# Z1HaoC/YOLO-Dual

Measured on AMD Instinct MI355X. Metric: images/sec at 640x640 bs=16/GPU, higher is better.
Workload: dtype bf16; 1 GPU; YOLOv5-backbone (C3+SPPF) + UNet-lite SegmentHead, fwd+bwd+SGD/EMA step, 640x640, bs=16/GPU, CE+0.5*Dice, 12 classes (BASELINE configs[1]); global_batch=16, parallelism=dp1

## Files before the change

yolo_dual_amd/csrc/igemm.hip:

```cpp
#include "conv_common.h"

#define GROWB 128


struct IgemmArgs {
    const void* A;
    const void* B;
    void* C;
    float* stats;
    int N, Hi, Wi, lda;
    int Kc;
    int Ho, Wo, ldc;
    int Cout;
    int Cst;
    int Hg, Wg;
    int in_mul, out_mul, out_h0, out_w0;
    int ntaps, Ttot;
    int accumulate;
    int M;
    int stats_ld;
    int stats_atomic;
    unsigned bytesA, bytesB;
    unsigned bytesC;
    unsigned ldb_bytes;
// ... 1167 lines not shown
#pragma unroll
            for (int j = 0; j < PT; ++j) bfr[j] = *(const uint4*)(pst + prow[j] * GROWB + ((kq ^ ((prow[j] >> 1) & 7)) << 4));
#pragma unroll
            for (int c = 0; c < CT; ++c)
#pragma unroll
                for (int j = 0; j < PT; ++j) Mma<T>::run(af[c], bfr[j], acc[c][j]);
        }
        stg = stg + 1 == S ? 0 : stg + 1;
    };
#define H_STEPS(F, CB)                                                                                                          \
    step(std::integral_constant<int, 0>{}, F, CB); step(std::integral_constant<int, 1>{}, F, CB);                              \
    step(std::integral_constant<int, 2>{}, F, CB); step(std::integral_constant<int, 3>{}, F, CB);                              \
    step(std::integral_constant<int, 4>{}, F, CB); step(std::integral_constant<int, 5>{}, F, CB);                              \
    step(std::integral_constant<int, 6>{}, F, CB); step(std::integral_constant<int, 7>{}, F, CB);                              \
    step(std::integral_constant<int, 8>{}, F, CB)
    H_STEPS(std::true_type{}, 0);
    for (int cb = 1; cb < spt; ++cb) { H_STEPS(std::false_type{}, cb); }
#undef H_STEPS
    asm volatile("s_waitcnt lgkmcnt(0)" ::: "memory");
    wait_vm_barrier<0>();
    igemm2_epilogue<BM, BN, NW, WP>(p, acc, smem, 0, n0, mtile, BM, 16, 8, n * p.Ho + h0, w0);
}

#define HS_PROWS 184
template <int BN, int NW, int WP, bool ONEP = false>
__global__ __launch_bounds__(NW * 64) void igemm2hs_kernel(const IgemmArgs p) {
    using T = bf16_t;
    constexpr int ES = 2;
    constexpr int BM = 128;
    constexpr int RPP = NW * 8;
    constexpr int BR = BN / RPP;
    constexpr int PP = (HS_PROWS + RPP - 1) / RPP;
    constexpr int WN = NW / WP;
    constexpr int BNW = BN / WN;
    constexpr int CT = BNW / 16;
    constexpr int PT = BM / (16 * WP);
    constexpr int PBYTES = HS_PROWS * GROWB;
    constexpr int RBYTES = BN * GROWB;
    static_assert(BN % RPP == 0 && (ONEP ? 1 : 2) * PBYTES + 2 * RBYTES >= BM * BN * 2 + 8192, "stage geometry");
    extern __shared__ __attribute__((aligned(16))) unsigned char smem[];
    constexpr int NPB = ONEP ? 1 : 2;
    unsigned char* const ring = smem + NPB * PBYTES;
    int* const sTd = (int*)(ring + 2 * RBYTES);
    int* const sTw = sTd + 16;
    const int t = threadIdx.x;
    if (t < 9) {
        sTd[t] = (int)p.dh[t] * H_PW + (int)p.dw[t];
        sTw[t] = (int)p.wt[t] * p.Kc * ES;
    }
    __syncthreads();
    const int lane = t & 63;
    const int wave = __builtin_amdgcn_readfirstlane(t >> 6);
    const int wc = wave % WN, wp = wave / WN;
    const int tile = xcd_remap(blockIdx.x, gridDim.x);
    int mtile, ntile;
    if (p.m_fastest) { ntile = tile / p.grid_m; mtile = tile - ntile * p.grid_m; }
    else { mtile = tile / p.grid_n; ntile = tile - mtile * p.grid_n; }
    const int tiles_w = p.Wo >> 4, tiles_hw = (p.Ho >> 3) * tiles_w;
    const int n = mtile / tiles_hw;
    const int rem = mtile - n * tiles_hw;
    const int h0 = (rem / tiles_w) << 3, w0 = (rem % tiles_w) << 4;
    const int n0 = ntile * BN;
    const int r = t >> 3, qs = t & 7;
    unsigned poff[PP];
#pragma unroll
    for (int i = 0; i < PP; ++i) {
        const int rho = r + RPP * i;
        const int pr = rho / H_PW, pc = rho - pr * H_PW;
        const int h = h0 - 1 + pr, w = w0 - 1 + pc;
        const bool ok = rho < 10 * H_PW && (unsigned)h < (unsigned)p.Hi && (unsigned)w < (unsigned)p.Wi;
        poff[i] = ok ? (unsigned)(((n * p.Hi + h) * p.Wi + w) * p.lda) * (unsigned)ES + (unsigned)((qs ^ ((rho >> 1) & 7)) << 4) : 0xFFFFFFFFu;
    }
    unsigned browoff[BR];
#pragma unroll
    for (int i = 0; i < BR; ++i) {
        const int row = r + RPP * i;
        const int co = n0 + row;
        browoff[i] = co < p.Cout ? (unsigned)co * p.ldb_bytes + (unsigned)((qs ^ ((row >> 1) & 7)) << 4) : 0xF0000000u;
    }
    const int spt = p.Kc >> 6;
    const int nsteps = 9 * spt;
    u32x4 rsA, rsB;
    ring_rsrc(p, rsA, rsB);
    const unsigned lds0 = (unsigned)(size_t)(__attribute__((address_space(3))) unsigned char*)smem;
    const unsigned wave_lds = lds0 + (unsigned)wave * (8 * GROWB);
    auto issue_patch = [&](int cb) {
        const unsigned base = wave_lds + (unsigned)(ONEP ? 0 : (cb & 1)) * PBYTES;
        const unsigned kb = (unsigned)cb << 7;
#pragma unroll
        for (int i = 0; i < PP; ++i) {
            if (RPP * i + wave * 8 < HS_PROWS)
                lds_dma16(rsA, base + i * RPP * GROWB, poff[i] == 0xFFFFFFFFu ? 0xFFFFFFFFu : poff[i] + kb);
        }
    };
    auto issue_w = [&](int stg, int cbw, int woff) {
        const unsigned add = cbw < spt ? (unsigned)woff + ((unsigned)cbw << 7) : 0xF0000000u;
        const unsigned base = wave_lds + (unsigned)NPB * PBYTES + (unsigned)stg * RBYTES;
#pragma unroll
        for (int i = 0; i < BR; ++i) lds_dma16(rsB, base + i * RPP * GROWB, browoff[i] + add);
    };
    f32x4 acc[CT][PT];
#pragma unroll
    for (int c = 0; c < CT; ++c)
#pragma unroll
        for (int j = 0; j < PT; ++j) acc[c][j] = f32x4{0.f, 0.f, 0.f, 0.f};
    const int lrow = lane & 15, lgrp = lane >> 4;
    const int sw_w = (lrow >> 1) & 7;
    const unsigned char* const fa = ring + (wc * BNW + lrow) * GROWB;
    issue_patch(0);
    issue_w(0, 0, sTw[0]);
    int cb = 0, tap = 0;
    int dcur = sTd[0], wnx = sTw[1];
    for (int g = 0; g < nsteps; ++g) {
        asm volatile("s_waitcnt lgkmcnt(0)" ::: "memory");
        wait_vm_barrier<0>();
        const int t1 = tap == 8 ? 0 : tap + 1, c1 = tap == 8 ? cb + 1 : cb;
        const int t2 = t1 == 8 ? 0 : t1 + 1;
        const int dnx = sTd[t1], wnn = sTw[t2];
        issue_w((g + 1) & 1, c1, wnx);
        if constexpr (ONEP) {
            if (tap == 0 && cb > 0) {
                issue_patch(cb);
                wait_vm_barrier<0>();
            }
        } else {
            if (tap == 0 && cb + 1 < spt) issue_patch(cb + 1);
        }
        const unsigned char* const wst = fa + (g & 1) * RBYTES;
        const unsigned char* const pst = smem + (ONEP ? 0 : (cb & 1)) * PBYTES;
        int prow[PT];
#pragma unroll
        for (int j = 0; j < PT; ++j) prow[j] = (wp * PT + j + 1) * H_PW + (lrow + 1) + dcur;
#pragma unroll
        for (int half = 0; half < 2; ++half) {
            uint4 af[CT], bfr[PT];
            const int kq = lgrp + 4 * half;
#pragma unroll
            for (int c = 0; c < CT; ++c) af[c] = *(const uint4*)(wst + c * 16 * GROWB + ((kq ^ sw_w) << 4));
#pragma unroll
            for (int j = 0; j < PT; ++j) bfr[j] = *(const uint4*)(pst + prow[j] * GROWB + ((kq ^ ((prow[j] >> 1) & 7)) << 4));
#pragma unroll
            for (int c = 0; c < CT; ++c)
#pragma unroll
                for (int j = 0; j < PT; ++j) Mma<T>::run(af[c], bfr[j], acc[c][j]);
        }
        dcur = dnx; wnx = wnn; tap = t1; cb = c1;
    }
    asm volatile("s_waitcnt lgkmcnt(0)" ::: "memory");
    wait_vm_barrier<0>();
    igemm2_epilogue<BM, BN, NW, WP>(p, acc, smem, 0, n0, mtile, BM, 16, 8, n * p.Ho + h0, w0);
}

#define WR_PW 34
typedef __attribute__((ext_vector_type(16))) float f32x16_t;
template <int CO, bool STATS, int NW>
__global__ __launch_bounds__(NW * 64, 2) void igemm2w_kernel(const IgemmArgs p, int nblocks) {
    using T = bf16_t;
    constexpr int CG = CO / 32, PG = NW / CG, RW = 2, R = PG * RW;
    constexpr int NT = NW * 64, PR = NW * 8;
    constexpr int PROWS = (R + 2) * WR_PW;
    constexpr int PASSES = (PROWS + PR - 1) / PR;
    constexpr int PBYTES = PASSES * PR * GROWB;
    constexpr int BPX = R * 32;
    constexpr int NCH = CO / 8;
    constexpr int ORB = CO * 2;
    static_assert(BPX * NCH == 4 * NT && NT % NCH == 0, "four 16-byte store slots per thread, a fixed channel chunk per thread");
    extern __shared__ __attribute__((aligned(16))) unsigned char smem[];
    unsigned char* const stage = smem + 2 * PBYTES;
    float* const sred = (float*)smem;
    const int t = threadIdx.x, lane = t & 63;
    const int wave = __builtin_amdgcn_readfirstlane(t >> 6);
    const int cg = wave % CG, pg = wave / CG;
    const int ln = lane & 31, lh = lane >> 5;
    const int blocks_w = p.Wo >> 5, blocks_img = (p.Ho / R) * blocks_w;
    const u32x4 rsA = buf_rsrc(p.A, p.bytesA), rsC = buf_rsrc(p.C, p.bytesC);
    const unsigned lds0 = (unsigned)(size_t)(__attribute__((address_space(3))) unsigned char*)smem;
    const unsigned wave_lds = lds0 + (unsigned)wave * 1024u;
    const int rq = t >> 3, qs = t & 7;
    int pprc[PASSES];
#pragma unroll
    for (int i = 0; i < PASSES; ++i) {
        const int rho = i * PR + rq;
        pprc[i] = rho < PROWS ? ((rho / WR_PW) << 8) | (rho - (rho / WR_PW) * WR_PW) : (4000000 << 8);
    }
    auto block_origin = [&](int b, int& n, int& h0, int& w0) {
        n = b / blocks_img;
        const int rem = b - n * blocks_img;
        h0 = (rem / blocks_w) * R;
        w0 = (rem % blocks_w) << 5;
    };
    auto issue_patch = [&](int b, int buf) {
        int n, h0, w0;
        block_origin(b, n, h0, w0);
        const bool live = b < nblocks;
#pragma unroll
        for (int i = 0; i < PASSES; ++i) {
            const int rho = i * PR + rq;
            const int h = h0 - 1 + (pprc[i] >> 8), w = w0 - 1 + (pprc[i] & 255);
            const bool ok = live && (unsigned)h < (unsigned)p.Hi && (unsigned)w < (unsigned)p.Wi;
            const unsigned off = (unsigned)(((n * p.Hi + h) * p.Wi + w) * p.lda) * 2u + (unsigned)((qs ^ ((rho >> 1) & 7)) << 4);
            lds_dma16(rsA, wave_lds + (unsigned)buf * PBYTES + (unsigned)(i * PR * GROWB), ok ? off : 0xFFFFFFFFu);
        }
    };
    const int per = (nblocks + (int)gridDim.x - 1) / (int)gridDim.x;
    const int b0 = blockIdx.x * per, b1 = min(nblocks, b0 + per);
    issue_patch(b0, 0);
    uint4 wreg[9][4];
    {
        const __amdgpu_buffer_rsrc_t rsB = __builtin_amdgcn_make_buffer_rsrc((void*)p.B, 0, p.bytesB, 0x00020000);
        const int co = cg * 32 + ln;
#pragma unroll
        for (int tp = 0; tp < 9; ++tp)
#pragma unroll
            for (int ks = 0; ks < 4; ++ks) {
                const unsigned off = co < p.Cout ? (unsigned)co * p.ldb_bytes + (unsigned)(((int)p.wt[tp] * p.Kc + ks * 16 + lh * 8) * 2) : 0xFFFFFFFFu;
                const u32x4 v = __builtin_amdgcn_raw_buffer_load_b128(rsB, off, 0, 0);
                wreg[tp][ks] = make_uint4(v.x, v.y, v.z, v.w);
            }
    }
    int tapd[9];
#pragma unroll
    for (int tp = 0; tp < 9; ++tp) tapd[tp] = (int)p.dh[tp] * WR_PW + (int)p.dw[tp];
    float s1[STATS ? 16 : 1], s2[STATS ? 16 : 1];
#pragma unroll
    for (int e = 0; e < (STATS ? 16 : 1); ++e) { s1[e] = 0.f; s2[e] = 0.f; }
    const bool want_stats = STATS && p.stats != nullptr;
    int ridx_base = (pg * RW + 1) * WR_PW + ln + 1;
    asm volatile("s_waitcnt vmcnt(0)\n\ts_barrier" ::: "memory");
    int buf = 0;
    for (int b = b0; b < b1; ++b, buf ^= 1) {
        issue_patch(b + 1 < b1 ? b + 1 : nblocks, buf ^ 1);
        const unsigned char* const pst = smem + buf * PBYTES;
        f32x16_t acc[RW];
#pragma unroll
        for (int rb = 0; rb < RW; ++rb)
#pragma unroll
            for (int e = 0; e < 16; ++e) acc[rb][e] = 0.f;
        asm volatile("" : "+v"(ridx_base));
        uint4 fq[2][4];
        auto rd = [&](int tp, int rb, uint4 (&f)[4]) {
            const int ridx = ridx_base + rb * WR_PW + tapd[tp];
            const unsigned char* const rowp = pst + ridx * GROWB;
            const int sw = (ridx >> 1) & 7;
#pragma unroll
            for (int ks = 0; ks < 4; ++ks) f[ks] = *(const uint4*)(rowp + (((2 * ks + lh) ^ sw) << 4));
        };
        rd(0, 0, fq[0]);
#pragma unroll
        for (int step = 0; step < 9 * RW; ++step) {
            const int tp = step / RW, rb = step % RW;
            if (step + 1 < 9 * RW) rd((step + 1) / RW, (step + 1) % RW, fq[(step + 1) & 1]);
#pragma unroll
            for (int ks = 0; ks < 4; ++ks)
                acc[rb] = __builtin_amdgcn_mfma_f32_32x32x16_bf16(__builtin_bit_cast(bf16x8, wreg[tp][ks]),
                                                                  __builtin_bit_cast(bf16x8, fq[step & 1][ks]), acc[rb], 0, 0, 0);
            __builtin_amdgcn_sched_barrier(0);
        }
        if constexpr (STATS) {
            if (want_stats) {
#pragma unroll
                for (int rb = 0; rb < RW; ++rb)
#pragma unroll
                    for (int e = 0; e < 16; ++e) { s1[e] += acc[rb][e]; s2[e] = fmaf(acc[rb][e], acc[rb][e], s2[e]); }
            }
        }
#pragma unroll
        for (int rb = 0; rb < RW; ++rb) {
            const int px = (pg * RW + rb) * 32 + ln;
#pragma unroll
            for (int g = 0; g < 4; ++g) {
                uint2 u;
                u.x = (uint32_t)f2bf(acc[rb][4 * g + 0]) | ((uint32_t)f2bf(acc[rb][4 * g + 1]) << 16);
                u.y = (uint32_t)f2bf(acc[rb][4 * g + 2]) | ((uint32_t)f2bf(acc[rb][4 * g + 3]) << 16);
                const int chq = cg * 4 + g;
                *(uint2*)(stage + px * ORB + ((chq ^ (px & (NCH - 1))) << 4) + (lh << 3)) = u;
            }
        }
        asm volatile("s_waitcnt lgkmcnt(0)\n\ts_barrier" ::: "memory");
        {
            int n, h0, w0;
            block_origin(b, n, h0, w0);
#pragma unroll
            for (int j = 0; j < 4; ++j) {
                const int idx = t + NT * j;
                const int px = idx / NCH, ch = idx % NCH;
                const uint4 v = *(const uint4*)(stage + px * ORB + ((ch ^ (px & (NCH - 1))) << 4));
                const unsigned m = (unsigned)((n * p.Ho + h0 + (px >> 5)) * p.Wo + w0 + (px & 31));
                const unsigned off = ch * 8 < p.Cst ? (m * (unsigned)p.ldc + (unsigned)(ch * 8)) * 2u : 0xFFFFFFFFu;
                asm volatile("s_waitcnt lgkmcnt(0)" ::: "memory");
                buf_store16_asm(u32x4{v.x, v.y, v.z, v.w}, off, rsC);
            }
        }
        asm volatile("s_waitcnt vmcnt(4)\n\ts_barrier" ::: "memory");
    }
    if constexpr (!STATS) {
        asm volatile("s_waitcnt vmcnt(0)" ::: "memory");
        return;
    }
    if (want_stats) {
#pragma unroll
        for (int e = 0; e < (STATS ? 16 : 1); ++e)
#pragma unroll
            for (int o = 1; o < 32; o <<= 1) { s1[e] += __shfl_xor(s1[e], o, 64); s2[e] += __shfl_xor(s2[e], o, 64); }
        asm volatile("s_waitcnt vmcnt(0) lgkmcnt(0)\n\ts_barrier" ::: "memory");
        if (ln == 0) {
#pragma unroll
            for (int e = 0; e < (STATS ? 16 : 1); ++e) {
                const int c = cg * 32 + (e >> 2) * 8 + lh * 4 + (e & 3);
                sred[(pg * CO + c) * 2] = s1[e];
                sred[(pg * CO + c) * 2 + 1] = s2[e];
            }
        }
        __syncthreads();
        if (t < CO && t < p.Cout) {
            float a = 0.f, b2 = 0.f;
#pragma unroll
            for (int w = 0; w < PG; ++w) { a += sred[(w * CO + t) * 2]; b2 += sred[(w * CO + t) * 2 + 1]; }
            float* dst = p.stats + (size_t)(blockIdx.x & (YDL_BN_REPLICAS - 1)) * 2 * p.stats_ld;
            atomicAdd(dst + t, a);
            atomicAdd(dst + p.stats_ld + t, b2);
        }
    } else {
        asm volatile("s_waitcnt vmcnt(0)" ::: "memory");
    }
}

static int g_wreg = 1;
static bool wreg_ok(const IgemmArgs& a) {
    if (!g_wreg || a.accumulate) return false;
    if (a.ncls > 1 || a.ntaps != 9 || a.Ttot != 9 || a.in_mul != 1 || a.out_mul != 1 || a.out_h0 != 0 || a.out_w0 != 0) return false;
    if (a.Hi != a.Ho || a.Wi != a.Wo || a.Hg != a.Ho || a.Wg != a.Wo || a.Kc != 64) return false;
    if (a.Cst != 64 && a.Cst != 128) return false;
    if ((a.Wo & 31) || a.Ho % (a.Cst == 128 ? 4 : 8)) return false;
    if (a.stats != nullptr && !a.stats_atomic) return false;
    if ((long long)a.M < 4ll * 128 * ydl_device_cus()) return false;
    bool seen[9] = {false, false, false, false, false, false, false, false, false};
    for (int t = 0; t < 9; ++t) {
        const int dh = a.dh[t], dw = a.dw[t];
        if (dh < -1 || dh > 1 || dw < -1 || dw > 1 || seen[(dh + 1) * 3 + dw + 1]) return false;
        seen[(dh + 1) * 3 + dw + 1] = true;
    }
    return true;
}
template <int CO>
static int launch_igemm2w_cfg(IgemmArgs a, hipStream_t st, int fam) {
    constexpr int NW = 4, R = (NW / (CO / 32)) * 2, PR = NW * 8;
    const int nblocks = a.N * (a.Ho / R) * (a.Wo >> 5);
    constexpr int PASSES = ((R + 2) * WR_PW + PR - 1) / PR;
    const size_t smem = 2 * (size_t)PASSES * PR * GROWB + (size_t)R * 32 * CO * 2;
    YDL_SET_MAX_LDS((igemm2w_kernel<CO, true, NW>), smem);
    YDL_SET_MAX_LDS((igemm2w_kernel<CO, false, NW>), smem);
    const unsigned long long bc = ((unsigned long long)(a.N * a.Ho * a.Wo - 1) * a.ldc + a.Cst) * 2ull;
    YDL_CHECK(bc < 0xFFFFFFF0ull, "output larger than 4 GiB");
    a.bytesC = (unsigned)bc;
    ydl_note_kernel(fam, CO == 128 ? "igemm2w_kernel<128,nw4>" : "igemm2w_kernel<64,nw4>");
    const int ctas = std::min(ydl_device_cus() * 2, nblocks);
    if (a.stats != nullptr) igemm2w_kernel<CO, true, NW><<<ctas, NW * 64, smem, st>>>(a, nblocks);
    else igemm2w_kernel<CO, false, NW><<<ctas, NW * 64, smem, st>>>(a, nblocks);
    YDL_LAUNCH_CHECK();
    return 0;
}
static int launch_igemm2w(const IgemmArgs& a, hipStream_t st, int fam) {
    return a.Cst == 128 ? launch_igemm2w_cfg<128>(a, st, fam) : launch_igemm2w_cfg<64>(a, st, fam);
}

#define S2_PW 17
#define S2_PROWS 192
__device__ constexpr int kS2Kh[9] = {1, 1, 2, 2, 1, 2, 0, 0, 0};
__device__ constexpr int kS2Kw[9] = {1, 2, 1, 2, 0, 0, 1, 2, 0};
template <int NW, int WP, int S, bool ACC>
__global__ __launch_bounds__(NW * 64, NW / 2) void igemm2s_kernel(const IgemmArgs p) {
    using T = bf16_t;
    constexpr int ES = 2;
    constexpr int BM = 128, BN = 64;
    constexpr int RPP = NW * 8;
    constexpr int BR = BN / RPP;
    constexpr int PP = (S2_PROWS + RPP - 1) / RPP;
    constexpr int WN = NW / WP;
    constexpr int BNW = BN / WN;
    constexpr int CT = BNW / 16;
    constexpr int PT = BM / (16 * WP);
    constexpr int PBYTES = S2_PROWS * GROWB;
    constexpr int RBYTES = BN * GROWB;
    static_assert(BN % RPP == 0 && BR == 1 && S2_PROWS % RPP == 0 && (S == 2 || S == 3), "one weight DMA per thread and step, whole patch passes");
    static_assert(2 * PBYTES + S * RBYTES >= BM * BN * 2, "epilogue scratch");
    extern __shared__ __attribute__((aligned(16))) unsigned char smem[];
    unsigned char* const ring = smem + 2 * PBYTES;
    const int t = threadIdx.x;
    const int lane = t & 63;
    const int wave = __builtin_amdgcn_readfirstlane(t >> 6);
    const int wc = wave % WN, wp = wave / WN;
    const int tile = xcd_remap(blockIdx.x, gridDim.x);
    const int mtile = tile / p.grid_n, ntile = tile - mtile * p.grid_n;
    const int tiles_w = p.Wi >> 4, tiles_hw = (p.Hi >> 3) * tiles_w;
    const int n = mtile / tiles_hw;
    const int rem = mtile - n * tiles_hw;
    const int i0 = (rem / tiles_w) << 3, j0 = (rem % tiles_w) << 4;
    const int n0 = ntile * BN;
    const int r = t >> 3, qs = t & 7;
    const unsigned browoff = (n0 + r) < p.Cout ? (unsigned)(n0 + r) * p.ldb_bytes + (unsigned)((qs ^ ((r >> 1) & 7)) << 4) : 0xF0000000u;
    const int spt = p.Kc >> 6;
    u32x4 rsA, rsB;
    ring_rsrc(p, rsA, rsB);
    const unsigned lds0 = (unsigned)(size_t)(__attribute__((address_space(3))) unsigned char*)smem;
    const unsigned wave_lds = lds0 + (unsigned)wave * (8 * GROWB);
    auto issue_patch = [&](int cb) {
        const unsigned base = wave_lds + (unsigned)(cb & 1) * PBYTES;
        const unsigned kb = (unsigned)cb << 7;
        const bool live = cb < spt;
#pragma unroll
        for (int i = 0; i < PP; ++i) {
            const int rho = r + RPP * i;
            const int pr = rho / S2_PW, pc = rho - pr * S2_PW;
            const int h = i0 + pr, w = j0 + pc;
            const bool ok = live && rho < 9 * S2_PW && h < p.Hi && w < p.Wi;
            const unsigned off = (unsigned)(((n * p.Hi + h) * p.Wi + w) * p.lda) * (unsigned)ES + (unsigned)((qs ^ ((rho >> 1) & 7)) << 4) + kb;
            lds_dma16(rsA, base + i * RPP * GROWB, ok ? off : 0xFFFFFFFFu);
        }
    };
    auto issue_w = [&](int stg, int cb, int slice) {
        const unsigned add = cb < spt ? (unsigned)slice * (unsigned)p.Kc * ES + ((unsigned)cb << 7) : 0xF0000000u;
        lds_dma16(rsB, wave_lds + 2u * PBYTES + (unsigned)stg * RBYTES, browoff + add);
    };
    f32x4 acc[4][CT][PT];
#pragma unroll
    for (int q = 0; q < 4; ++q)
#pragma unroll
        for (int c = 0; c < CT; ++c)
#pragma unroll
            for (int j = 0; j < PT; ++j) acc[q][c][j] = f32x4{0.f, 0.f, 0.f, 0.f};
    const int lrow = lane & 15, lgrp = lane >> 4;
    const int sw_w = (lrow >> 1) & 7;
    const unsigned char* const fa = ring + (wc * BNW + lrow) * GROWB;
    uint4 bq[2][PT];
    auto step = [&](auto ic, int cb) {
        constexpr int I = decltype(ic)::value;
        constexpr int kh = kS2Kh[I], kw = kS2Kw[I];
        constexpr int dh = kh == 0 ? 1 : 0, dw = kw == 0 ? 1 : 0;
        constexpr int cls = (kh != 1 ? 2 : 0) + (kw != 1 ? 1 : 0);
        constexpr bool group_start = I == 0 || I == 4 || I == 6 || I == 8;
        constexpr int I1 = (I + 8) % 9, I2 = (I + 7) % 9;
        constexpr int NY = S == 2 ? 0 : 1 + (I1 == 0 ? PP : 0) + (I2 == 0 ? PP : 0);
        asm volatile("s_waitcnt lgkmcnt(0)" ::: "memory");
        wait_vm_barrier<NY>();
        {
            constexpr int J = (I + S - 1) % 9;
            const int cbj = cb + (I + S - 1) / 9;
            issue_w(S == 3 ? J % 3 : (cbj + J) & 1, cbj, kS2Kh[J] * 3 + kS2Kw[J]);
        }
        if constexpr (I == 0) issue_patch(cb + 1);
        const unsigned char* const wst = fa + (S == 3 ? I % 3 : (cb + I) & 1) * RBYTES;
        const unsigned char* const pst = smem + (cb & 1) * PBYTES;
        if constexpr (group_start) {
#pragma unroll
            for (int j = 0; j < PT; ++j) {
                const int prow = (wp * PT + j + dh) * S2_PW + (lrow + dw);
                const unsigned char* const rowp = pst + prow * GROWB;
                const int sw = (prow >> 1) & 7;
                bq[0][j] = *(const uint4*)(rowp + ((lgrp ^ sw) << 4));
                bq[1][j] = *(const uint4*)(rowp + (((lgrp + 4) ^ sw) << 4));
            }
        }
#pragma unroll
        for (int half = 0; half < 2; ++half) {
            uint4 aq[CT];
#pragma unroll
            for (int c = 0; c < CT; ++c) aq[c] = *(const uint4*)(wst + c * 16 * GROWB + (((lgrp + 4 * half) ^ sw_w) << 4));
#pragma unroll
            for (int c = 0; c < CT; ++c)
#pragma unroll
                for (int j = 0; j < PT; ++j) Mma<T>::run(aq[c], bq[half][j], acc[cls][c][j]);
        }
    };
    issue_patch(0);
    issue_w(0, 0, kS2Kh[0] * 3 + kS2Kw[0]);
    if constexpr (S == 3) issue_w(1, 0, kS2Kh[1] * 3 + kS2Kw[1]);
    for (int cb = 0; cb < spt; ++cb) {
        step(std::integral_constant<int, 0>{}, cb); step(std::integral_constant<int, 1>{}, cb); step(std::integral_constant<int, 2>{}, cb);
        step(std::integral_constant<int, 3>{}, cb); step(std::integral_constant<int, 4>{}, cb); step(std::integral_constant<int, 5>{}, cb);
        step(std::integral_constant<int, 6>{}, cb); step(std::integral_constant<int, 7>{}, cb); step(std::integral_constant<int, 8>{}, cb);
    }
    asm volatile("s_waitcnt lgkmcnt(0)" ::: "memory");
    wait_vm_barrier<0>();
    if constexpr (ACC) {
        constexpr int CPR = BN / 8, RPS = NW * 64 / CPR, ORB = BN * 2;
        static_assert(4 * BM * ORB <= 2 * PBYTES + S * RBYTES && CPR == 8, "the four previous tiles must fit the LDS");
        const u32x4 rsC = buf_rsrc(p.C, p.bytesC);
#pragma unroll
        for (int q = 0; q < 4; ++q)
#pragma unroll
            for (int i = 0; i < BM / RPS; ++i) {
                const int row = r + i * RPS;
                const int gh = row >> 4, gw = row & 15;
                const unsigned pix = (unsigned)((n * p.Ho + 2 * (i0 + gh) + (q >> 1)) * p.Wo + 2 * (j0 + gw) + (q & 1));
                const int co = n0 + ((qs ^ (row & 7)) << 3);
                lds_dma16(rsC, wave_lds + (unsigned)(q * BM * ORB + i * RPS * ORB), co < p.Cst ? (pix * (unsigned)p.ldc + (unsigned)co) * ES : 0xFFFFFFFFu);
                __builtin_amdgcn_sched_barrier(0);
            }
        wait_vm_barrier<0>();
#pragma unroll
        for (int q = 0; q < 4; ++q)
#pragma unroll
            for (int j = 0; j < PT; ++j) {
                const int row = wp * (BM / WP) + j * 16 + lrow;
#pragma unroll
                for (int c = 0; c < CT; ++c) {
                    const int ch = wc * BNW + c * 16 + lgrp * 4;
                    const uint2 q2 = *(const uint2*)(smem + q * BM * ORB + row * ORB + ((((ch >> 3) ^ (row & 7))) << 4) + ((ch & 4) << 1));
                    acc[q][c][j] += f32x4{__uint_as_float(q2.x << 16), __uint_as_float(q2.x & 0xffff0000u),
                                          __uint_as_float(q2.y << 16), __uint_as_float(q2.y & 0xffff0000u)};
                }
                __builtin_amdgcn_sched_barrier(0);
            }
        __syncthreads();
    }
// ... 630 lines not shown
}

template <int BM, int BN, int NW, int WP, int S, int NL>
static int launch_igemm2l(IgemmArgs a, hipStream_t st, int fam) {
    if (int e = ring_grid(a, BM, BN)) return e;
    const size_t smem = (size_t)S * (BM + BN) * GROWB + 3 * MAXTAPS * sizeof(int);
    static const std::string nm = std::string("igemm2l_kernel<") + std::to_string(BM) + "," + std::to_string(BN) + "," + std::to_string(NW) + "+" +
                                  std::to_string(NL) + "," + std::to_string(S) + ">";
    YDL_SET_MAX_LDS((igemm2l_kernel<BM, BN, NW, WP, S, NL>), smem);
    ydl_note_kernel(fam, nm.c_str());
    igemm2l_kernel<BM, BN, NW, WP, S, NL><<<dim3(a.grid_m * a.grid_n), (NW + NL) * 64, smem, st>>>(a);
    YDL_LAUNCH_CHECK();
    return 0;
}

static int g_halo = 1;
static bool halo_ok(const IgemmArgs& a, int id) {
    if (!g_halo || !kRing[id].patch) return false;
    if (a.ncls > 1 || a.ntaps != 9 || a.Ttot != 9 || a.in_mul != 1 || a.out_mul != 1 || a.out_h0 != 0 || a.out_w0 != 0) return false;
    if (a.Hi != a.Ho || a.Wi != a.Wo || a.Hg != a.Ho || a.Wg != a.Wo || (a.Ho & 7) || (a.Wo & 15) || (a.Kc & 63)) return false;
    bool seen[9] = {false, false, false, false, false, false, false, false, false};
    for (int t = 0; t < 9; ++t) {
        const int dh = a.dh[t], dw = a.dw[t];
        if (dh < -1 || dh > 1 || dw < -1 || dw > 1 || seen[(dh + 1) * 3 + dw + 1]) return false;
        seen[(dh + 1) * 3 + dw + 1] = true;
    }
    return true;
}
template <int BN, int S>
static int launch_igemm2h(IgemmArgs a, hipStream_t st, int fam) {
    constexpr int NW = 8, WP = 4;
    if (int e = ring_grid(a, 128, BN)) return e;
    static const std::string nm = std::string("igemm2h_kernel<128,") + std::to_string(BN) + "," + std::to_string(S) + ">";
    ydl_note_kernel(fam, nm.c_str());
    if constexpr (S == 2) {
        if (a.Kc == 64) {
            const size_t smem = (size_t)HS_PROWS * GROWB + 2 * (size_t)BN * GROWB + 128;
            YDL_SET_MAX_LDS((igemm2hs_kernel<BN, NW, WP, true>), smem);
            igemm2hs_kernel<BN, NW, WP, true><<<dim3(a.grid_m * a.grid_n), NW * 64, smem, st>>>(a);
        } else {
            const size_t smem = 2 * (size_t)HS_PROWS * GROWB + 2 * (size_t)BN * GROWB + 128;
            YDL_SET_MAX_LDS((igemm2hs_kernel<BN, NW, WP>), smem);
            igemm2hs_kernel<BN, NW, WP><<<dim3(a.grid_m * a.grid_n), NW * 64, smem, st>>>(a);
        }
    } else {
        const size_t smem = 2 * (size_t)H_PROWS * GROWB + (size_t)S * BN * GROWB;
        YDL_SET_MAX_LDS((igemm2h_kernel<BN, NW, WP, S>), smem);
        igemm2h_kernel<BN, NW, WP, S><<<dim3(a.grid_m * a.grid_n), NW * 64, smem, st>>>(a);
    }
    YDL_LAUNCH_CHECK();
    return 0;
}
static int launch_patch(int id, const IgemmArgs& a, hipStream_t st, int fam) {
    if (kRing[id].BN == 128) return launch_igemm2h<128, 2>(a, st, fam);
    if (a.Kc == 64) return launch_igemm2h<64, 2>(a, st, fam);
    return launch_igemm2h<64, 3>(a, st, fam);
}

static int g_s2fused = 1;
static bool s2fused_ok(const ydl_conv_geom* g, int dtype) {
    if (!g_s2fused || !g_ring_enabled || dtype != YDL_BF16) return false;
    if (g->k != 3 || g->s != 2 || g->p != 1 || g->Hi != 2 * g->Ho || g->Wi != 2 * g->Wo) return false;
    if ((g->Ho & 7) || (g->Wo & 15) || (round_up(g->Cout, 8) & 63) || (g->Cin & 7) || g->Cin < 64) return false;
    return true;
}
template <bool ACC>
static int launch_igemm2s_cfg(const IgemmArgs& a, hipStream_t st, int fam) {
    constexpr int NW = 8, WP = 4, S = 2;
    const size_t smem = 2 * (size_t)S2_PROWS * GROWB + (size_t)S * 64 * GROWB;
    YDL_SET_MAX_LDS((igemm2s_kernel<NW, WP, S, ACC>), smem);
    ydl_note_kernel(fam, ACC ? "igemm2s_kernel<128,64,2,acc>" : "igemm2s_kernel<128,64,2>");
    igemm2s_kernel<NW, WP, S, ACC><<<dim3(a.grid_m * a.grid_n), NW * 64, smem, st>>>(a);
    YDL_LAUNCH_CHECK();
    return 0;
}
static int launch_igemm2s(IgemmArgs a, hipStream_t st, int fam) {
    if (int e = check_ring_weights(a)) return e;
    a.grid_n = (a.Cst + 63) / 64;
    a.grid_m = a.N * (a.Hi >> 3) * (a.Wi >> 4);
    return a.accumulate ? launch_igemm2s_cfg<true>(a, st, fam) : launch_igemm2s_cfg<false>(a, st, fam);
}

static int launch_ring(int id, const IgemmArgs& a, hipStream_t st, int fam) {
    if (a.br.nseg > 0) {
        switch (id) {
            case RING_128x128: return launch_igemm2<128, 128, 8, 4, 2, true>(a, st, fam);
            case RING_64x128: return launch_igemm2<64, 128, 4, 2, 3, true>(a, st, fam);
            case RING_128x64: return launch_igemm2<128, 64, 8, 4, 2, true>(a, st, fam);
        }
        ydl_set_error("fused BatchNorm reduce: no instantiation for this ring configuration (query ydl_conv_dgrad_bnred_supported)");
        return 1;
    }
    switch (id) {
        case RING_128x128: return launch_igemm2<128, 128, 8, 4, 2>(a, st, fam);
        case RING_64x128: return launch_igemm2<64, 128, 4, 2, 3>(a, st, fam);
        case RING_128x64: return launch_igemm2<128, 64, 8, 4, 2>(a, st, fam);
        case RING_256x128_STG: return launch_igemm2<256, 128, 8, 4, 3, false, 1>(a, st, fam);
        case RING_256x128_LOADERS: return launch_igemm2l<256, 128, 8, 4, 3, 4>(a, st, fam);
        case RING_128x128_LOADERS: return launch_igemm2l<128, 128, 8, 4, 3, 4>(a, st, fam);
        case RING_128x128_LOADERS_S2: return launch_igemm2l<128, 128, 4, 2, 2, 4>(a, st, fam);
    }
    ydl_set_error("internal: unknown ring kernel id");
    return 1;
}

static TileCfg pick_cfg(int M, int Cst, int nchunks, bool bf16, int Kc, int taps, bool one_class, bool loaders_ok) {
    TileCfg c;
    c.ring = RING_NONE;
    if (bf16 && g_ring_enabled && Cst >= 64 && Cst % 8 == 0 && nchunks >= 16 && Kc > 0 && Kc % 64 == 0 && taps <= 29) {
        const long b128 = (long)((M + 127) / 128) * ((Cst + 127) / 128);
        int id = b128 < 256 ? RING_64x128 : RING_128x128;
        const long b256 = (long)((M + 255) / 256) * ((Cst + 127) / 128);
        if (one_class && Cst >= 128 && b256 >= 180 && b256 <= 512 && nchunks >= 96) id = RING_256x128_STG;
        if (g_ring_loaders && loaders_ok) {
            if (id == RING_256x128_STG && nchunks >= 128) id = RING_256x128_LOADERS;
            if (id == RING_64x128 && b128 >= 64) id = RING_128x128_LOADERS;
            if (id == RING_128x128 && b128 < 1280) id = RING_128x128_LOADERS_S2;
        }
        if (Cst < 128) id = RING_128x64;
        c.ring = id; c.BM = kRing[id].BM; c.BN = kRing[id].BN;
        return c;
    }
    c.BN = Cst <= 16 ? 16 : (Cst <= 64 ? 64 : 128);
    c.BM = 128;
    long blocks = (long)((M + 127) / 128) * ((Cst + c.BN - 1) / c.BN);
    if (blocks < 512 && c.BN == 128) {
        long b1 = (long)((M + 127) / 128) * ((Cst + 63) / 64);
        if (b1 >= 512) { c.BN = 64; return c; }
    }
    if (blocks < 512 && c.BN != 16) c.BM = 64;
    if (c.BM == 64 && c.BN == 128) {
        long b2 = (long)((M + 63) / 64) * ((Cst + 127) / 128);
        if (b2 < 512) c.BN = 64;
    }
    return c;
}

enum ConvFamily { CONV_STEM, CONV_PW, CONV_WREG, CONV_PATCH, CONV_RING, CONV_TILE };
struct ConvPlan {
    ConvFamily family;
    TileCfg tile;
    PwPlan pw;
    int grid_m, block_m;
    bool has_bnred;
};
static ConvPlan conv_plan(const IgemmArgs& a, int es, int fam, bool with_reduce) {
    ConvPlan pl{};
    if (es == 2 && fam == 0 && args_stem(a)) {
        const StemPlan sp = stem_plan(a.M, a.Wo);
        if (sp.ok) { pl.family = CONV_STEM; pl.grid_m = sp.grid_m; pl.block_m = sp.block_m; return pl; }
    }
    pl.pw = pw_plan(a.M, a.Kc, a.Cout, a.Cst, es, args_pointwise(a));
    if (pl.pw.ok) { pl.family = CONV_PW; pl.grid_m = pl.pw.grid_m; pl.block_m = pl.pw.block_m; return pl; }
    if (es == 2 && !with_reduce && wreg_ok(a)) { pl.family = CONV_WREG; return pl; }
    int nch = a.ntaps * (a.Kc / (16 / es));
    if (a.ncls > 1) {
        nch = 1 << 30;
        for (int i = 0; i < a.ncls; ++i) nch = min(nch, a.cls_ntaps[i] * (a.Kc / (16 / es)));
    }
    pl.tile = pick_cfg(a.M, a.Cst, nch, es == 2, a.Kc, a.Ttot, a.ncls <= 1, !with_reduce);
    pl.block_m = pl.tile.BM;
    pl.family = CONV_TILE;
    if (pl.tile.ring) {
        const bool patch = !with_reduce && halo_ok(a, pl.tile.ring);
        pl.family = patch ? CONV_PATCH : CONV_RING;
        if (patch) pl.block_m = 128;
        pl.has_bnred = !patch && ring_has_bnred(pl.tile.ring);
    }
    pl.grid_m = (a.M + pl.block_m - 1) / pl.block_m;
    return pl;
}

template <typename T>
static int dispatch_igemm(const IgemmArgs& a, hipStream_t st, int fam) {
    const ConvPlan pl = conv_plan(a, (int)sizeof(T), fam, a.br.nseg > 0);
    switch (pl.family) {
        case CONV_STEM: {
            StemArgs q{};
            q.X = (const bf16_t*)a.A; q.W = (const bf16_t*)a.B; q.Y = (bf16_t*)a.C; q.stats = a.stats;
            q.H = a.Hi; q.Wd = a.Wi; q.ldc = a.ldc; q.M = a.M; q.block_m = pl.block_m; q.stats_ld = a.stats_ld;
            q.stats_atomic = a.stats_atomic; q.bytesX = a.bytesA;
            ydl_note_kernel(fam, "stem_kernel<bf16,16,64>");
            stem_kernel<<<pl.grid_m, 256, 0, st>>>(q);
            YDL_LAUNCH_CHECK();
            return 0;
        }
        case CONV_PW: {
            YDL_CHECK(a.br.nseg == 0, "fused BatchNorm reduce: this geometry runs on the point-wise kernel (query ydl_conv_dgrad_bnred_supported)");
            PwArgs q{};
            q.X = a.A; q.W = a.B; q.Y = a.C; q.stats = a.stats;
            q.M = a.M; q.lda = a.lda; q.ldc = a.ldc; q.Cout = a.Cout; q.WN = pl.pw.WN; q.accumulate = a.accumulate;
            q.block_m = pl.pw.block_m; q.stats_ld = a.stats_ld; q.stats_atomic = a.stats_atomic; q.bytesX = a.bytesA; q.ldw_bytes = a.ldb_bytes;
            return launch_pw<T>(q, pl.pw, st, fam);
        }
        case CONV_WREG: return launch_igemm2w(a, st, fam);
        case CONV_PATCH: return launch_patch(pl.tile.ring, a, st, fam);
        case CONV_RING: return launch_ring(pl.tile.ring, a, st, fam);
        case CONV_TILE: break;
    }
    YDL_CHECK(a.br.nseg == 0, "fused BatchNorm reduce: this geometry runs on the register-staged kernel (query ydl_conv_dgrad_bnred_supported)");
    const TileCfg& c = pl.tile;
    if (c.BM == 128 && c.BN == 128) return launch_igemm<T, 128, 128, 8>(a, st, fam);
    if (c.BM == 128 && c.BN == 64) return launch_igemm<T, 128, 64>(a, st, fam);
    if (c.BM == 128 && c.BN == 16) return launch_igemm<T, 128, 16>(a, st, fam);
    if (c.BM == 64 && c.BN == 128) return launch_igemm<T, 64, 128, 8>(a, st, fam);
    if (c.BM == 64 && c.BN == 64) return launch_igemm<T, 64, 64>(a, st, fam);
    return launch_igemm<T, 64, 16>(a, st, fam);
}

static int set_extents(IgemmArgs& a, int dtype) {
    const unsigned long long es = (unsigned long long)esize(dtype);
    unsigned long long ba = (unsigned long long)a.N * a.Hi * a.Wi * a.lda * es;
    if (a.ldb_bytes == 0) a.ldb_bytes = (unsigned)((unsigned long long)a.Ttot * a.Kc * es);
    unsigned long long bb = (unsigned long long)(a.Cout - 1) * a.ldb_bytes + (unsigned long long)a.Ttot * a.Kc * es;
    YDL_CHECK(ba < 0xFFFFFFF0ull && bb < 0xFFFFFFF0ull, "tensor larger than 4 GiB: not addressable by the 32-bit buffer loads");
    a.bytesA = (unsigned)ba;
    a.bytesB = (unsigned)bb;
    return 0;
}


static int fwd_args(const ydl_conv_geom* g, int dtype, const void* x, const void* w, void* y, float* stats_ws, int stats_atomic,
                    int accumulate, IgemmArgs& a) {
    if (int e = check_geom(g, dtype)) return e;
    a = IgemmArgs{};
    a.A = x; a.B = w; a.C = y; a.stats = stats_ws;
    a.N = g->N; a.Hi = g->Hi; a.Wi = g->Wi; a.lda = g->ldx;
    a.Kc = round_up(g->Cin, 8);
    a.Ho = g->Ho; a.Wo = g->Wo; a.ldc = g->ldy; a.Cout = g->Cout;
    a.Cst = round_up(g->Cout, 8) <= g->ldy ? round_up(g->Cout, 8) : g->Cout;
    a.Hg = g->Ho; a.Wg = g->Wo; a.in_mul = g->s; a.out_mul = 1; a.out_h0 = 0; a.out_w0 = 0;
    a.ntaps = g->k * g->k; a.Ttot = a.ntaps; a.accumulate = accumulate ? 1 : 0;
    a.M = g->N * g->Ho * g->Wo;
    a.stats_ld = round_up(g->Cout, 8);
    a.stats_atomic = stats_atomic;
    a.ldb_bytes = (unsigned)(g->ldw * esize(dtype));
    for (int r = 0; r < g->k; ++r)
        for (int s = 0; s < g->k; ++s) {
            int tpi = r * g->k + s;
            a.dh[tpi] = (signed char)(r - g->p); a.dw[tpi] = (signed char)(s - g->p); a.wt[tpi] = (unsigned char)tpi;
        }
    return set_extents(a, dtype);
}

static ConvPlan fwd_blocks(const ydl_conv_geom* g, int dtype) {
    static float stats_tag;
    IgemmArgs a;
    if (fwd_args(g, dtype, nullptr, nullptr, nullptr, &stats_tag, 0, 0, a)) return ConvPlan{};
    return conv_plan(a, esize(dtype), 0, false);
}

extern "C" int64_t ydl_conv_fwd_stats_ws_bytes(const ydl_conv_geom* g, int dtype) {
    const ConvPlan r = fwd_blocks(g, dtype);
    if (r.grid_m <= 0) return 0;
    return ((int64_t)r.grid_m + r.grid_m / 64 + 2) * 2 * round_up(g->Cout, 8) * (int64_t)sizeof(float);
}
extern "C" int ydl_conv_fwd_grid_m(const ydl_conv_geom* g, int dtype) { return fwd_blocks(g, dtype).grid_m; }
extern "C" int ydl_conv_fwd_block_m(const ydl_conv_geom* g, int dtype) { return fwd_blocks(g, dtype).block_m; }

static int conv_fwd_impl(const ydl_conv_geom* g, int dtype, const void* x, const void* w, void* y,
                         float* stats_ws, int stats_atomic, int accumulate, void* stream) {
    IgemmArgs a;
    if (int e = fwd_args(g, dtype, x, w, y, stats_ws, stats_atomic, accumulate, a)) return e;
    YDL_CHECK(aligned16(x) && aligned16(w) && aligned16(y), "pointers must be 16-byte aligned");
    if (stats_ws != nullptr && !stats_atomic && accumulate) {
        IgemmArgs a0 = a;
        a0.accumulate = 0;
        const ConvPlan r0 = conv_plan(a0, esize(dtype), 0, false), r1 = conv_plan(a, esize(dtype), 0, false);
        YDL_CHECK(r0.grid_m == r1.grid_m && r0.block_m == r1.block_m,
                  "partial-row statistics with accumulate != 0: this geometry runs on another kernel than ydl_conv_fwd_grid_m / _block_m describe");
    }
    hipStream_t st = (hipStream_t)stream;
    return dtype == YDL_F32 ? dispatch_igemm<float>(a, st, 0) : dispatch_igemm<bf16_t>(a, st, 0);
}

extern "C" int ydl_conv_fwd(const ydl_conv_geom* g, int dtype, const void* x, const void* w, void* y,
                            float* stats_ws, int accumulate, void* stream) {
    return conv_fwd_impl(g, dtype, x, w, y, stats_ws, 0, accumulate, stream);
}
extern "C" int ydl_conv_fwd_sums(const ydl_conv_geom* g, int dtype, const void* x, const void* w, void* y,
                                 float* sums, int accumulate, void* stream) {
    YDL_CHECK(sums != nullptr, "null sums");
    return conv_fwd_impl(g, dtype, x, w, y, sums, 1, accumulate, stream);
}

static int conv_dgrad_impl(const ydl_conv_geom* g, int dtype, const void* dy, const void* wt, void* dx,
                           int accumulate, const ydl_bnred* red, ConvPlan* plan_out, void* stream) {
    if (int e = check_geom(g, dtype)) return e;
    YDL_CHECK(plan_out || (aligned16(dy) && aligned16(wt) && aligned16(dx)), "pointers must be 16-byte aligned");
    YDL_CHECK(g->ldy >= round_up(g->Cout, 8), "dy pixel stride must cover Cout rounded up to 8");
    hipStream_t st = (hipStream_t)stream;
    const int s = g->s, k = g->k, pd = g->p;
    struct Cls { int ph, pw, nt, Hg, Wg; signed char dh[MAXTAPS], dw[MAXTAPS]; unsigned char wt[MAXTAPS]; };
    static thread_local Cls cls[16];
    int ncls = 0, total_taps = 0;
    YDL_CHECK(s * s <= 16, "stride too large for the dgrad class table");
    for (int ph = 0; ph < s; ++ph)
        for (int pw = 0; pw < s; ++pw) {
            Cls& c = cls[ncls];
            c.ph = ph; c.pw = pw;
            c.Hg = (g->Hi - ph + s - 1) / s; c.Wg = (g->Wi - pw + s - 1) / s;
            if (c.Hg <= 0 || c.Wg <= 0) continue;
            int nt = 0;
            for (int r = 0; r < k; ++r) {
                int nh = ph + pd - r;
                if (((nh % s) + s) % s != 0) continue;
                for (int cc = 0; cc < k; ++cc) {
                    int nw = pw + pd - cc;
                    if (((nw % s) + s) % s != 0) continue;
                    int dh = nh >= 0 ? nh / s : -((-nh) / s), dw = nw >= 0 ? nw / s : -((-nw) / s);
                    c.dh[nt] = (signed char)dh; c.dw[nt] = (signed char)dw; c.wt[nt] = (unsigned char)(r * k + cc);
                    ++nt;
                }
            }
            c.nt = nt;
            total_taps += nt;
            ++ncls;
        }
    auto base_args = [&]() {
        IgemmArgs a{};
        a.A = dy; a.B = wt; a.C = dx; a.stats = nullptr;
        a.N = g->N; a.Hi = g->Ho; a.Wi = g->Wo; a.lda = g->ldy;
        a.Kc = round_up(g->Cout, 8);
        a.Ho = g->Hi; a.Wo = g->Wi; a.ldc = g->ldx; a.Cout = g->Cin;
        a.Cst = g->Cin;
        a.in_mul = 1; a.out_mul = s;
        a.Ttot = k * k; a.accumulate = accumulate;
        if (red) a.br = *red;
        return a;
    };
    auto run = [&](const IgemmArgs& a) -> int {
        if (plan_out) { *plan_out = conv_plan(a, esize(dtype), 1, true); return 0; }
        return dtype == YDL_F32 ? dispatch_igemm<float>(a, st, 1) : dispatch_igemm<bf16_t>(a, st, 1);
    };
    if (red == nullptr && plan_out == nullptr && ncls == 4 && s2fused_ok(g, dtype)) {
        IgemmArgs a = base_args();
        a.M = g->N * g->Ho * g->Wo; a.Hg = g->Ho; a.Wg = g->Wo; a.ntaps = 9;
        if (int e2 = set_extents(a, dtype)) return e2;
        const unsigned long long bc = (unsigned long long)g->N * g->Hi * g->Wi * g->ldx * 2ull;
        if (bc < 0xFFFFFFF0ull) {
            a.bytesC = (unsigned)bc;
            return launch_igemm2s(a, st, 1);
        }
    }
    if (g_dgrad_merge && ncls > 1 && ncls <= 4 && total_taps <= MAXTAPS) {
        int order[4] = {0, 1, 2, 3};
        for (int i = 0; i < ncls; ++i)
            for (int j = i + 1; j < ncls; ++j)
                if (cls[order[j]].nt > cls[order[i]].nt) { int t = order[i]; order[i] = order[j]; order[j] = t; }
        IgemmArgs a = base_args();
        a.ncls = ncls;
        int tp = 0;
        for (int i = 0; i < ncls; ++i) {
            const Cls& c = cls[order[i]];
            a.cls_ntaps[i] = c.nt; a.cls_tap0[i] = tp; a.cls_Hg[i] = c.Hg; a.cls_Wg[i] = c.Wg;
            a.cls_M[i] = g->N * c.Hg * c.Wg; a.cls_h0[i] = c.ph; a.cls_w0[i] = c.pw;
            for (int t = 0; t < c.nt; ++t) { a.dh[tp + t] = c.dh[t]; a.dw[tp + t] = c.dw[t]; a.wt[tp + t] = c.wt[t]; }
            tp += c.nt;
        }
        a.Hg = a.cls_Hg[0]; a.Wg = a.cls_Wg[0]; a.out_h0 = a.cls_h0[0]; a.out_w0 = a.cls_w0[0];
        a.ntaps = a.cls_ntaps[0];
        a.M = 0;
        for (int i = 0; i < ncls; ++i) a.M += a.cls_M[i];
        if (int e2 = set_extents(a, dtype)) return e2;
        return run(a);
    }
    if (plan_out && ncls > 1) { *plan_out = ConvPlan{}; plan_out->family = CONV_TILE; return 0; }
    YDL_CHECK(red == nullptr || ncls == 1, "fused BatchNorm reduce needs the single-launch dgrad");
    for (int ci = 0; ci < ncls; ++ci) {
        const Cls& c = cls[ci];
        IgemmArgs a = base_args();
        a.Hg = c.Hg; a.Wg = c.Wg; a.out_h0 = c.ph; a.out_w0 = c.pw;
        a.M = g->N * a.Hg * a.Wg;
        a.ntaps = c.nt;
        for (int t = 0; t < c.nt; ++t) { a.dh[t] = c.dh[t]; a.dw[t] = c.dw[t]; a.wt[t] = c.wt[t]; }
        if (int e2 = set_extents(a, dtype)) return e2;
        if (int e = run(a)) return e;
    }
    return 0;
}

extern "C" int ydl_conv_dgrad(const ydl_conv_geom* g, int dtype, const void* dy, const void* wt, void* dx,
                              int accumulate, void* stream) {
    return conv_dgrad_impl(g, dtype, dy, wt, dx, accumulate, nullptr, nullptr, stream);
}

extern "C" int ydl_conv_dgrad_bnred_supported(const ydl_conv_geom* g, int dtype) {
    if (g == nullptr || dtype != YDL_BF16) return 0;
    ConvPlan pl{};
    if (conv_dgrad_impl(g, dtype, nullptr, nullptr, nullptr, 0, nullptr, &pl, nullptr) != 0) return 0;
    return pl.family == CONV_RING && pl.has_bnred ? 1 : 0;
}

extern "C" int ydl_conv_dgrad_bnred(const ydl_conv_geom* g, int dtype, const void* dy, const void* wt, void* dx,
                                    int accumulate, const ydl_bnred* red, void* stream) {
    YDL_CHECK(red != nullptr && (red->nseg == 1 || red->nseg == 2), "one or two channel segments");
    YDL_CHECK(dtype == YDL_BF16, "the fused reduce exists for bf16 only");
    for (int i = 0; i < red->nseg; ++i) {
        YDL_CHECK(red->c0[i] >= 0 && red->c0[i] < red->c1[i] && red->c0[i] % 8 == 0 && red->c1[i] % 8 == 0 && red->c1[i] <= round_up(g->Cin, 8),
                  "segment channel range must be 8-aligned inside the gradient's channels");
        YDL_CHECK(red->cp[i] >= red->c1[i] - red->c0[i] && red->ldy[i] >= red->c1[i] - red->c0[i], "segment strides too small");
        YDL_CHECK(red->y[i] && red->scale[i] && red->shift[i] && red->mean[i] && red->invstd[i] && red->sums[i], "null segment pointer");
        YDL_CHECK(aligned16(red->y[i]) && (red->ldy[i] * 2) % 16 == 0, "segment y must be 16-byte aligned");
        YDL_CHECK(red->act[i] == YDL_ACT_NONE || red->act[i] == YDL_ACT_SILU, "segment activation: none or SiLU");
    }
    YDL_CHECK(red->nseg == 1 || red->c1[0] <= red->c0[1], "segments must be ordered and disjoint");
    return conv_dgrad_impl(g, dtype, dy, wt, dx, accumulate, red, nullptr, stream);
}

extern int g_resize_int, g_resize_rows;
void ydl_dcn_debug_set(int key, int val);
void ydl_deform_debug_set(int key, int val);
void ydl_wgrad_debug_set(int key, int val);
extern "C" void ydl_debug_set(int key, int val) {
    ydl_dcn_debug_set(key, val);
    ydl_deform_debug_set(key, val);
    ydl_wgrad_debug_set(key, val);
    if (key == 1) g_pw_enabled = val;
    if (key == 2) g_dgrad_merge = val;
    if (key == 3) g_ring_enabled = val;
    if (key == 5) g_stem_enabled = val;
    if (key == 6) g_ring_persist = val;
    if (key == 8) g_halo = val;
    if (key == 9) g_s2fused = val;
    if (key == 10) g_resize_int = val;
    if (key == 11) g_resize_rows = val;
    if (key == 14) g_pw_acc_ts = val;
    if (key == 17) g_wreg = val;
    if (key == 19) g_ring_loaders = val;
}
```

Measured before the change: 2692 images/sec.

## Extend register-resident-weight 3x3 conv kernel to stride-2 forward convs

Generalizes the weight-in-register igemm2w kernel to handle stride-2 3x3 convolutions with 64 input channels and 128 outputs. It uses a de-interleaved patch layout (even columns, then odd columns) so each tap reads contiguous LDS rows, and adds a single-buffer mode to fit the larger patch in LDS. Stride-2 forward convs with BN stats then use this kernel instead of the generic tiled path. The trade-off is lost prefetch overlap (no double buffering) and larger patch loads per block.

```diff
diff --git a/yolo_dual_amd/csrc/igemm.hip b/yolo_dual_amd/csrc/igemm.hip
--- a/yolo_dual_amd/csrc/igemm.hip
+++ b/yolo_dual_amd/csrc/igemm.hip
@@ -1343,13 +1343,16 @@
 }
 
 #define WR_PW 34
+#define WR_PW2 66
 typedef __attribute__((ext_vector_type(16))) float f32x16_t;
-template <int CO, bool STATS, int NW>
+template <int CO, bool STATS, int NW, int S = 1, int NBUF = 2>
 __global__ __launch_bounds__(NW * 64, 2) void igemm2w_kernel(const IgemmArgs p, int nblocks) {
     using T = bf16_t;
     constexpr int CG = CO / 32, PG = NW / CG, RW = 2, R = PG * RW;
     constexpr int NT = NW * 64, PR = NW * 8;
-    constexpr int PROWS = (R + 2) * WR_PW;
+    constexpr int PW = S == 2 ? WR_PW2 : WR_PW;
+    constexpr int PROWS = (S == 2 ? 2 * R + 1 : R + 2) * PW;
+    static_assert((S == 1 || S == 2) && (NBUF == 1 || NBUF == 2), "stride 1 or 2, one or two patch buffers");
     constexpr int PASSES = (PROWS + PR - 1) / PR;
     constexpr int PBYTES = PASSES * PR * GROWB;
     constexpr int BPX = R * 32;
@@ -1357,7 +1360,7 @@
     constexpr int ORB = CO * 2;
     static_assert(BPX * NCH == 4 * NT && NT % NCH == 0, "four 16-byte store slots per thread, a fixed channel chunk per thread");
     extern __shared__ __attribute__((aligned(16))) unsigned char smem[];
-    unsigned char* const stage = smem + 2 * PBYTES;
+    unsigned char* const stage = smem + NBUF * PBYTES;
     float* const sred = (float*)smem;
     const int t = threadIdx.x, lane = t & 63;
     const int wave = __builtin_amdgcn_readfirstlane(t >> 6);
@@ -1368,11 +1371,15 @@
     const unsigned lds0 = (unsigned)(size_t)(__attribute__((address_space(3))) unsigned char*)smem;
     const unsigned wave_lds = lds0 + (unsigned)wave * 1024u;
     const int rq = t >> 3, qs = t & 7;
-    int pprc[PASSES];
-#pragma unroll
-    for (int i = 0; i < PASSES; ++i) {
-        const int rho = i * PR + rq;
-        pprc[i] = rho < PROWS ? ((rho / WR_PW) << 8) | (rho - (rho / WR_PW) * WR_PW) : (4000000 << 8);
+    auto patch_rc = [](int rho) {
+        const int prow = rho / PW, slot = rho - prow * PW;
+        const int pcol = S == 2 ? (slot < 33 ? 2 * slot : 2 * (slot - 33) + 1) : slot;
+        return rho < PROWS ? (prow << 8) | pcol : (4000000 << 8);
+    };
+    int pprc[S == 1 ? PASSES : 1];
+    if constexpr (S == 1) {
+#pragma unroll
+        for (int i = 0; i < PASSES; ++i) pprc[i] = patch_rc(i * PR + rq);
     }
     auto block_origin = [&](int b, int& n, int& h0, int& w0) {
         n = b / blocks_img;
@@ -1384,10 +1391,13 @@
         int n, h0, w0;
         block_origin(b, n, h0, w0);
         const bool live = b < nblocks;
+        int rqv = rq;
+        if constexpr (S == 2) asm volatile("" : "+v"(rqv));
 #pragma unroll
         for (int i = 0; i < PASSES; ++i) {
-            const int rho = i * PR + rq;
-            const int h = h0 - 1 + (pprc[i] >> 8), w = w0 - 1 + (pprc[i] & 255);
+            const int rho = i * PR + rqv;
+            const int prc = S == 1 ? pprc[S == 1 ? i : 0] : patch_rc(rho);
+            const int h = S * h0 - 1 + (prc >> 8), w = S * w0 - 1 + (prc & 255);
             const bool ok = live && (unsigned)h < (unsigned)p.Hi && (unsigned)w < (unsigned)p.Wi;
             const unsigned off = (unsigned)(((n * p.Hi + h) * p.Wi + w) * p.lda) * 2u + (unsigned)((qs ^ ((rho >> 1) & 7)) << 4);
             lds_dma16(rsA, wave_lds + (unsigned)buf * PBYTES + (unsigned)(i * PR * GROWB), ok ? off : 0xFFFFFFFFu);
@@ -1411,16 +1421,19 @@
     }
     int tapd[9];
 #pragma unroll
-    for (int tp = 0; tp < 9; ++tp) tapd[tp] = (int)p.dh[tp] * WR_PW + (int)p.dw[tp];
+    for (int tp = 0; tp < 9; ++tp) {
+        const int dw = (int)p.dw[tp];
+        tapd[tp] = (int)p.dh[tp] * PW + (S == 2 ? (dw == 0 ? 33 : (dw > 0 ? 1 : 0)) : dw);
+    }
     float s1[STATS ? 16 : 1], s2[STATS ? 16 : 1];
 #pragma unroll
     for (int e = 0; e < (STATS ? 16 : 1); ++e) { s1[e] = 0.f; s2[e] = 0.f; }
     const bool want_stats = STATS && p.stats != nullptr;
-    int ridx_base = (pg * RW + 1) * WR_PW + ln + 1;
+    int ridx_base = (pg * RW * S + 1) * PW + ln + (S == 2 ? 0 : 1);
     asm volatile("s_waitcnt vmcnt(0)\n\ts_barrier" ::: "memory");
     int buf = 0;
-    for (int b = b0; b < b1; ++b, buf ^= 1) {
-        issue_patch(b + 1 < b1 ? b + 1 : nblocks, buf ^ 1);
+    for (int b = b0; b < b1; ++b, buf ^= NBUF - 1) {
+        if constexpr (NBUF == 2) issue_patch(b + 1 < b1 ? b + 1 : nblocks, buf ^ 1);
         const unsigned char* const pst = smem + buf * PBYTES;
         f32x16_t acc[RW];
 #pragma unroll
@@ -1430,7 +1443,7 @@
         asm volatile("" : "+v"(ridx_base));
         uint4 fq[2][4];
         auto rd = [&](int tp, int rb, uint4 (&f)[4]) {
-            const int ridx = ridx_base + rb * WR_PW + tapd[tp];
+            const int ridx = ridx_base + rb * (S * PW) + tapd[tp];
             const unsigned char* const rowp = pst + ridx * GROWB;
             const int sw = (ridx >> 1) & 7;
 #pragma unroll
@@ -1468,12 +1481,15 @@
             }
         }
         asm volatile("s_waitcnt lgkmcnt(0)\n\ts_barrier" ::: "memory");
+        if constexpr (NBUF == 1) issue_patch(b + 1 < b1 ? b + 1 : nblocks, 0);
         {
             int n, h0, w0;
             block_origin(b, n, h0, w0);
+            int ts = t;
+            if constexpr (S == 2) asm volatile("" : "+v"(ts));
 #pragma unroll
             for (int j = 0; j < 4; ++j) {
-                const int idx = t + NT * j;
+                const int idx = ts + NT * j;
                 const int px = idx / NCH, ch = idx % NCH;
                 const uint4 v = *(const uint4*)(stage + px * ORB + ((ch ^ (px & (NCH - 1))) << 4));
                 const unsigned m = (unsigned)((n * p.Ho + h0 + (px >> 5)) * p.Wo + w0 + (px & 31));
@@ -1517,13 +1533,16 @@
 }
 
 static int g_wreg = 1;
+static int g_wreg_s2 = 1;
 static bool wreg_ok(const IgemmArgs& a) {
-    if (!g_wreg || a.accumulate) return false;
-    if (a.ncls > 1 || a.ntaps != 9 || a.Ttot != 9 || a.in_mul != 1 || a.out_mul != 1 || a.out_h0 != 0 || a.out_w0 != 0) return false;
-    if (a.Hi != a.Ho || a.Wi != a.Wo || a.Hg != a.Ho || a.Wg != a.Wo || a.Kc != 64) return false;
-    if (a.Cst != 64 && a.Cst != 128) return false;
+    const int S = a.in_mul;
+    if (!g_wreg || a.accumulate || (S == 2 && !g_wreg_s2)) return false;
+    if (a.ncls > 1 || a.ntaps != 9 || a.Ttot != 9 || (S != 1 && S != 2) || a.out_mul != 1 || a.out_h0 != 0 || a.out_w0 != 0) return false;
+    if (a.Hi != S * a.Ho || a.Wi != S * a.Wo || a.Hg != a.Ho || a.Wg != a.Wo || a.Kc != 64) return false;
+    if (a.Cst != 128 && (a.Cst != 64 || S == 2)) return false;
     if ((a.Wo & 31) || a.Ho % (a.Cst == 128 ? 4 : 8)) return false;
     if (a.stats != nullptr && !a.stats_atomic) return false;
+    if (S == 2 && a.stats == nullptr) return false;
     if ((long long)a.M < 4ll * 128 * ydl_device_cus()) return false;
     bool seen[9] = {false, false, false, false, false, false, false, false, false};
     for (int t = 0; t < 9; ++t) {
@@ -1551,7 +1570,23 @@
     YDL_LAUNCH_CHECK();
     return 0;
 }
+static int launch_igemm2w_s2(IgemmArgs a, hipStream_t st, int fam) {
+    constexpr int CO = 128, NW = 4, NBUF = 1, R = (NW / (CO / 32)) * 2, PR = NW * 8;
+    const int nblocks = a.N * (a.Ho / R) * (a.Wo >> 5);
+    constexpr int PASSES = ((2 * R + 1) * WR_PW2 + PR - 1) / PR;
+    const size_t smem = NBUF * (size_t)PASSES * PR * GROWB + (size_t)R * 32 * CO * 2;
+    YDL_SET_MAX_LDS((igemm2w_kernel<CO, true, NW, 2, NBUF>), smem);
+    const unsigned long long bc = ((unsigned long long)(a.N * a.Ho * a.Wo - 1) * a.ldc + a.Cst) * 2ull;
+    YDL_CHECK(bc < 0xFFFFFFF0ull, "output larger than 4 GiB");
+    a.bytesC = (unsigned)bc;
+    ydl_note_kernel(fam, "igemm2w_kernel<128,s2,nw4>");
+    const int ctas = std::min(ydl_device_cus() * 2, nblocks);
+    igemm2w_kernel<CO, true, NW, 2, NBUF><<<ctas, NW * 64, smem, st>>>(a, nblocks);
+    YDL_LAUNCH_CHECK();
+    return 0;
+}
 static int launch_igemm2w(const IgemmArgs& a, hipStream_t st, int fam) {
+    if (a.in_mul == 2) return launch_igemm2w_s2(a, st, fam);
     return a.Cst == 128 ? launch_igemm2w_cfg<128>(a, st, fam) : launch_igemm2w_cfg<64>(a, st, fam);
 }
 
@@ -2488,7 +2523,7 @@
     }
     pl.pw = pw_plan(a.M, a.Kc, a.Cout, a.Cst, es, args_pointwise(a));
     if (pl.pw.ok) { pl.family = CONV_PW; pl.grid_m = pl.pw.grid_m; pl.block_m = pl.pw.block_m; return pl; }
-    if (es == 2 && !with_reduce && wreg_ok(a)) { pl.family = CONV_WREG; return pl; }
+    if (es == 2 && !with_reduce && (a.in_mul == 1 || fam == 0) && wreg_ok(a)) { pl.family = CONV_WREG; return pl; }
     int nch = a.ntaps * (a.Kc / (16 / es));
     if (a.ncls > 1) {
         nch = 1 << 30;
@@ -2764,4 +2799,5 @@
     if (key == 14) g_pw_acc_ts = val;
     if (key == 17) g_wreg = val;
     if (key == 19) g_ring_loaders = val;
-}
+    if (key == 21) g_wreg_s2 = val;
+}
```

Result: no change. 2697 images/sec, median of 6 (+0.2%).
